# reinterpretcat/qwen3-rs

Hardware: AMD Instinct MI355X
Metric: decode tokens/sec Qwen3-0.6B Q8 g=64 @1 GPU; % of int8 HBM roofline (higher is better)
Workload: dtype i8 (int8 x int8 -> i32 group dots, f32 scales/accumulate); 1 GPU; qwen3-0.6b Q8 group=64 single-stream greedy decode, 8-token prompt, reference generate-mode call pattern (first forward at pos 7, zero KV prefix), ctx 3072, 2751 tokens; mode=reference summation order (bit-identical logits), replicas=1, checkpoint_seed=1234

## Files before the change

qwen3-rs_amd/csrc/q3_attn_short2.h:

```cpp
#if defined(__HIP_DEVICE_COMPILE__) && !defined(__gfx950__)
#error "k_attn_short2 relies on gfx950 s_barrier behaviour for terminated waves; validated on gfx950 only"
#endif
constexpr int kS2Threads = 512;
constexpr int kS2MaxT = 256;
__host__ __device__ inline size_t attn_short2_smem_bytes(int hd, int max_t) { return 4 * (size_t)max_t * (size_t)(hd + 4); }

template <int V> struct IntC { static constexpr int value = V; };

#ifdef Q3_DEV
#define ATT2_STAMP(i, thr) do { if (a.stamps != nullptr && (a.debug & 64) == 0 && blockIdx.x == 3 && (int)threadIdx.x == (thr)) a.stamps[i] = __builtin_amdgcn_s_memtime(); } while (0)
#else
#define ATT2_STAMP(i, thr) do { } while (0)
#endif

template <int HD>
__global__ __launch_bounds__(kS2Threads) void k_attn_short2(const AttnArgs a) {
    static_assert(HD == 128, "head dim instantiated");
    constexpr int NQ4 = HD / 4;
    constexpr int HALF = HD / 2;
    constexpr int LD = HD + 4;
    constexpr int VT = 64;
    extern __shared__ __attribute__((aligned(16))) float ptile[];
    float* const vtile = ptile + VT * LD;
    __shared__ __attribute__((aligned(16))) float q_s[HD];
    __shared__ __attribute__((aligned(16))) float sq_s[2 * HD];
    __shared__ __attribute__((aligned(16))) float att[kS2MaxT];
    __shared__ __attribute__((aligned(16))) float att_e[kS2MaxT];
    __shared__ __attribute__((aligned(16))) float att_p[kS2MaxT];
    __shared__ unsigned long long etab[32];
    __shared__ unsigned vflag;
    __shared__ unsigned bcount;
    ATT2_STAMP(0, 0);
    KSTAMP_BEGIN(a);
    Q3_PIN_S(a.st); Q3_PIN_S(a.pos_override); Q3_PIN_S(a.q); Q3_PIN_S(a.k_raw); Q3_PIN_S(a.key_cache); Q3_PIN_S(a.value_cache);
    Q3_PIN_S(a.q_norm_w); Q3_PIN_S(a.k_norm_w); Q3_PIN_S(a.rope); Q3_PIN_S(a.xb); Q3_PIN_S(a.n_heads); Q3_PIN_S(a.n_kv_heads);
    Q3_PIN_S(a.write_q);

    const int kv_mul = a.kv_mul, xq = (int)((blockIdx.x * a.kvh_magic) >> 20);
    const int kvh = (int)blockIdx.x - xq * a.n_kv_heads;
    const int h = kvh * kv_mul + xq;
    const int tid = threadIdx.x, lane = tid & 63;
    const int wave = __builtin_amdgcn_readfirstlane(tid >> 6);
    const size_t kvd = (size_t)a.n_kv_heads * HD;
    const int pos_v = a.pos_override >= 0 ? a.pos_override : a.st->pos;
    const float* kbase = a.key_cache + (size_t)kvh * HD;
    const float* vbase = a.value_cache + (size_t)kvh * HD;

    if (wave == 4 || wave == 5) {
        const int pos = __builtin_amdgcn_readfirstlane(pos_v);
        const int np = pos + 1;
        const bool vsplit = gridDim.y == 2 && np > 64;
        if (gridDim.y == 2 && blockIdx.y == 1 && np <= 64) return;
        if (vsplit && wave == 5) {
            __syncthreads();
            __syncthreads();
            if (np > 128) __syncthreads();
            __syncthreads();
            return;
        }
        const int e = vsplit ? 64 * (int)blockIdx.y + lane : 64 * (wave - 4) + lane;
        const unsigned eoff = 4u * (unsigned)e;
        float vv[kShortVSets][32];
        auto v_issue = [&](float (&R)[32], int c) {
#pragma unroll
            for (int u = 0; u < 32; ++u) R[u] = *(const float*)((const char*)(vbase + (size_t)min(32 * c + u, pos) * kvd) + eoff);
        };
        auto v_pull = [&](float (&R)[32], int c) {
            const float* vp = vtile + e;
#pragma unroll
            for (int u = 0; u < 32; ++u) R[u] = vp[min(32 * c + u, pos) * HD];
        };
        const bool vlds = np <= VT;
        if (tid == 256) { vflag = 0u; bcount = 0u; }
        if (!vlds) {
#pragma unroll
            for (int c = 0; c < 2; ++c) v_issue(vv[c], c);
        }
        __syncthreads();
        if (!vlds) {
#pragma unroll
            for (int c = 2; c < kShortVSets; ++c)
                if (32 * c < np) v_issue(vv[c], c);
        }
        __syncthreads();
        if (vlds) {
            while (__hip_atomic_load(&vflag, __ATOMIC_ACQUIRE, __HIP_MEMORY_SCOPE_WORKGROUP) < 4u) __builtin_amdgcn_s_sleep(1);
#pragma unroll
            for (int c = 0; c < VT / 32; ++c)
                if (32 * c < np) v_pull(vv[c], c);
        }
        if (np > 128) __syncthreads();
        __syncthreads();
        ATT2_STAMP(5, 256);
        const v4f e4 = ((const v4f*)att_e)[lane];
        float sum;
        if (np <= 128) {
            sum = seq_chain(-0.0f, (const v4f*)att_e, (((np + 3) >> 2) + 7) & ~7);
        } else {
            const float etot = (e4.x + e4.y) + (e4.z + e4.w);
            sum = spec_sum_lanes(etot, (np + 3) >> 2, [&](float s) { return chain4(s, e4); });
        }
        ATT2_STAMP(13, 256);
        const float inv = 1.0f / sum;
        v4f p4;
        p4.x = e4.x * inv; p4.y = e4.y * inv; p4.z = e4.z * inv; p4.w = e4.w * inv;
        ((v4f*)att_p)[lane] = p4;
        wave_lds_sync();
        float o = 0.0f;
        auto fold_chunk = [&](const float (&R)[32], int c) {
            const v4f* pp = (const v4f*)att_p + 8 * c;
            v4f pq[8];
#pragma unroll
            for (int u4 = 0; u4 < 8; ++u4) pq[u4] = pp[u4];
#pragma unroll
            for (int u4 = 0; u4 < 8; ++u4) {
                if (32 * c + 4 * u4 < np) {
                    const v4f pv = pq[u4];
                    const v2f t01 = (v2f){pv.x, pv.y} * (v2f){R[4 * u4 + 0], R[4 * u4 + 1]};
                    const v2f t23 = (v2f){pv.z, pv.w} * (v2f){R[4 * u4 + 2], R[4 * u4 + 3]};
                    o = o + t01.x;
                    o = o + t01.y;
                    o = o + t23.x;
                    o = o + t23.y;
                }
            }
        };
#pragma unroll
        for (int c = 0; c < kShortVSets; ++c)
            if (32 * c < np) fold_chunk(vv[c], c);
        for (int c = kShortVSets; 32 * c < np; c += 2) {
            v_issue(vv[0], c);
            if (32 * (c + 1) < np) v_issue(vv[1], c + 1);
            fold_chunk(vv[0], c);
            if (32 * (c + 1) < np) fold_chunk(vv[1], c + 1);
        }
        ATT2_STAMP(14, 256);
        a.xb[(size_t)h * HD + e] = o;
        if (a.xbq != nullptr) {
            const float m = group_max_f32(fabsf(o), a.xb_group);
            const float scale = m / 127.0f;
            const int qv = (scale != 0.0f) ? quant_round_i8(o / scale) : 0;
            const int idx = h * HD + e;
            a.xbq[idx] = (int8_t)qv;
            if ((idx & (a.xb_group - 1)) == 0) a.xbs[idx / a.xb_group] = scale;
        }
        ATT2_STAMP(6, 256);
        KSTAMP_END(a);
        return;
    }

    int pos, np;
    if (wave < 2) {
        const bool is_q = wave == 0;
        const float* rawp = is_q ? a.q + (size_t)h * HD : a.k_raw + (size_t)kvh * HD;
        const float r_lo = rawp[lane], r_hi = rawp[lane + HALF];
        const float* nw = is_q ? a.q_norm_w : a.k_norm_w;
        const float w_lo = nw[lane], w_hi = nw[lane + HALF];
        __builtin_amdgcn_sched_barrier(0);
        pos = __builtin_amdgcn_readfirstlane(pos_v);
        np = pos + 1;
        if (gridDim.y == 2 && blockIdx.y == 1 && np <= 64) return;
        const v2f cs = *(const v2f*)(a.rope + (size_t)pos * HD + 2 * lane);
        ATT2_STAMP(1, 0);
        float* sq = sq_s + (is_q ? 0 : HD);
        sq[lane] = r_lo * r_lo;
        sq[lane + HALF] = r_hi * r_hi;
        wave_lds_sync();
        const float ss = seq_chain(-0.0f, (const v4f*)sq, NQ4);
        const float f = 1.0f / sqrtf(ss / (float)HD + kEps);
        const float xv = w_lo * (f * r_lo);
        const float yv = w_hi * (f * r_hi);
        const float a0 = xv * cs.x, b0 = yv * cs.y;
        const float a1 = xv * cs.y, b1 = yv * cs.x;
        const float lo = a0 - b0, hi = a1 + b1;
        if (is_q) {
            q_s[lane] = lo;
            q_s[lane + HALF] = hi;
            if (a.write_q) {
                a.q[(size_t)h * HD + lane] = lo;
                a.q[(size_t)h * HD + lane + HALF] = hi;
            }
        } else if ((h % kv_mul) == 0 && blockIdx.y == 0) {
            float* krow = a.key_cache + (size_t)pos * kvd + (size_t)kvh * HD;
            krow[lane] = lo;
            krow[lane + HALF] = hi;
        }
        ATT2_STAMP(2, 0);
        __syncthreads();
        if (!is_q) {
            ptile[pos * LD + lane] = q_s[lane] * lo;
            ptile[pos * LD + lane + HALF] = q_s[lane + HALF] * hi;
        }
    } else {
        unsigned long long etv = 0ull;
        if (wave == 7 && lane < 32) etv = kExp2Tab[lane];
#ifdef Q3_DEV
        const int hint = a.row_steps;
#else
        constexpr int hint = 0;
#endif
        if (hint <= 0) {
            pos = __builtin_amdgcn_readfirstlane(pos_v);
            np = pos + 1;
            if (gridDim.y == 2 && blockIdx.y == 1 && np <= 64) return;
        }
        ATT2_STAMP(8, 128);
        const int sidx = 64 * ((wave & 1) + (wave >= 6 ? 2 : 0)) + lane;
        const int r0 = sidx >> 5, col = sidx & 31;
        const unsigned loff = 4u * ((unsigned)r0 * (unsigned)kvd + 4u * (unsigned)col);
        const int kmax = max(a.seq_len / 8 - 1, 0);
        float* lp = ptile + r0 * LD + 4 * col;
        float* lv = vtile + r0 * HD + 4 * col;
        auto stage = [&](auto tier, auto with_v) {
            constexpr int T = decltype(tier)::value;
            constexpr bool V = decltype(with_v)::value != 0;
            v4f rk[T], rv[V ? T : 1];
#pragma unroll
            for (int k = 0; k < T; ++k) rk[k] = *(const v4f*)((const char*)(kbase + (size_t)min(k, kmax) * 8 * kvd) + loff);
            __builtin_amdgcn_sched_barrier(0);
            if constexpr (V) {
#pragma unroll
                for (int k = 0; k < T; ++k) rv[k] = *(const v4f*)((const char*)(vbase + (size_t)min(k, kmax) * 8 * kvd) + loff);
            }
            ATT2_STAMP(9, 128);
            if (hint > 0) {
                pos = __builtin_amdgcn_readfirstlane(pos_v);
                np = pos + 1;
            }
            __syncthreads();
            const v4f qv = ((const v4f*)q_s)[col];
#pragma unroll
            for (int k = 0; k < T; ++k) {
                const v2f p01 = (v2f){qv.x, qv.y} * (v2f){rk[k].x, rk[k].y};
                const v2f p23 = (v2f){qv.z, qv.w} * (v2f){rk[k].z, rk[k].w};
                v4f pr; pr.x = p01.x; pr.y = p01.y; pr.z = p23.x; pr.w = p23.y;
                if (r0 + 8 * k < pos) *(v4f*)(lp + 8 * k * LD) = pr;
            }
            if (wave == 7 && lane < 32) etab[lane] = etv;
            ATT2_STAMP(11, 128);
            if constexpr (V) {
                __syncthreads();
#pragma unroll
                for (int k = 0; k < T; ++k)
                    if (r0 + 8 * k < np) *(v4f*)(lv + 8 * k * HD) = rv[k];
                __builtin_amdgcn_fence(__ATOMIC_RELEASE, "workgroup");
                if (lane == 0) __hip_atomic_fetch_add(&vflag, 1u, __ATOMIC_RELAXED, __HIP_MEMORY_SCOPE_WORKGROUP);
                ATT2_STAMP(10, 128);
            }
        };
        const int tn = hint > 0 ? hint : (pos + 8) >> 3;
        if (tn <= 1) stage(IntC<1>{}, IntC<1>{});
        else if (tn <= 2) stage(IntC<2>{}, IntC<1>{});
        else if (tn <= 3) stage(IntC<3>{}, IntC<1>{});
        else if (tn <= 4) stage(IntC<4>{}, IntC<1>{});
        else if (tn <= 6) stage(IntC<6>{}, IntC<1>{});
        else if (tn <= 8) stage(IntC<8>{}, IntC<1>{});
        else if (tn <= 12) stage(IntC<12>{}, IntC<0>{});
        else if (tn <= 16) stage(IntC<16>{}, IntC<0>{});
        else if (tn <= 24) stage(IntC<24>{}, IntC<0>{});
        else stage(IntC<32>{}, IntC<0>{});
        if (np <= VT) return;
        __syncthreads();
        if (wave >= 6 || np <= 128) return;
    }
    if (wave < 2) __syncthreads();
    ATT2_STAMP(3, 0);

    const int t = 64 * wave + lane;
    float sc = -__builtin_inff();
    if (64 * wave < np) {
        const float scale = 1.0f / sqrtf((float)HD);
        const v4f* pr = (const v4f*)(ptile + min(t, pos) * LD);
        float dot = -0.0f;
        v4f pa[8], pb[8];
#pragma unroll
        for (int u = 0; u < 8; ++u) pa[u] = pr[u];
#pragma unroll
        for (int b = 0; b < NQ4 / 8; ++b) {
            if (b + 1 < NQ4 / 8) {
#pragma unroll
                for (int u = 0; u < 8; ++u) pb[u] = pr[8 * (b + 1) + u];
                __builtin_amdgcn_s_waitcnt(0xC87F);
            } else {
                __builtin_amdgcn_s_waitcnt(0xC07F);
            }
            __builtin_amdgcn_sched_barrier(0);
#pragma unroll
            for (int u = 0; u < 8; ++u) dot = chain4(dot, pa[u]);
            __builtin_amdgcn_sched_barrier(0);
#pragma unroll
            for (int u = 0; u < 8; ++u) pa[u] = pb[u];
        }
        sc = t < np ? dot * scale : -__builtin_inff();
    }
    const bool one_wave = np <= 64;
    float m;
    if (!one_wave) {
        att[t] = sc;
        if (np <= 128) {
            att[t + 128] = -__builtin_inff();
            __builtin_amdgcn_fence(__ATOMIC_RELEASE, "workgroup");
            if (lane == 0) {
                __hip_atomic_fetch_add(&bcount, 1u, __ATOMIC_RELAXED, __HIP_MEMORY_SCOPE_WORKGROUP);
                while (__hip_atomic_load(&bcount, __ATOMIC_RELAXED, __HIP_MEMORY_SCOPE_WORKGROUP) < 2u) __builtin_amdgcn_s_sleep(1);
            }
            __builtin_amdgcn_fence(__ATOMIC_ACQUIRE, "workgroup");
        } else {
            __syncthreads();
        }
        ATT2_STAMP(4, 0);
        const v4f s4 = ((const v4f*)att)[lane];
        m = fmaxf(fmaxf(s4.x, s4.y), fmaxf(s4.z, s4.w));
    } else {
        ATT2_STAMP(4, 0);
        m = sc;
    }
    m = group_max_f32(m, 64);
    float ev = 0.0f;
    if (64 * wave < np) {
        ev = q3_expf_wave(t < np ? sc - m : 0.0f, etab);
        ev = t < np ? ev : 0.0f;
    }
    att_e[t] = ev;
    if (np <= 128) att_e[t + 128] = 0.0f;
    __syncthreads();
    KSTAMP_END(a);
}
```

Measured before the change: 1130 tokens/s.

## Software-pipeline attention PV fold and exact-length softmax sum in short kernel

Restructures the short-context attention PV accumulation into a compile-time walk. Products for the next V chunk are computed while the previous chunk's sequential add chain runs, and probability loads and late V loads are issued ahead with explicit waitcnt and sched barriers. The softmax denominator now uses an exact-length sequential chain with a handled remainder and double-buffered LDS reads, where before it was padded to a multiple of eight. The q write-back is moved to the kernel tail and limited to blockIdx.y==0. This aims to hide LDS and global load latency and trim wasted adds, at the cost of more registers and more code complexity.

```diff
diff --git a/qwen3-rs_amd/csrc/q3_attn_short2.h b/qwen3-rs_amd/csrc/q3_attn_short2.h
--- a/qwen3-rs_amd/csrc/q3_attn_short2.h
+++ b/qwen3-rs_amd/csrc/q3_attn_short2.h
@@ -6,6 +6,56 @@
 __host__ __device__ inline size_t attn_short2_smem_bytes(int hd, int max_t) { return 4 * (size_t)max_t * (size_t)(hd + 4); }
 
 template <int V> struct IntC { static constexpr int value = V; };
+
+template <int MAXB>
+__device__ __forceinline__ float seq_chain_rem(float s, const v4f* p, int nq) {
+    const int nb = nq >> 3;
+    const v4f* pw = p + (nq & 7);
+    v4f buf[2][8];
+    auto head = [&](auto tc) {
+        constexpr int T = decltype(tc)::value;
+        v4f h[T > 0 ? T : 1];
+#pragma unroll
+        for (int k = 0; k < T; ++k) h[k] = p[k];
+        if (nb > 0) {
+#pragma unroll
+            for (int k = 0; k < 8; ++k) buf[0][k] = pw[k];
+            if constexpr (T > 0) __builtin_amdgcn_s_waitcnt(0xC87F);
+        } else {
+            __builtin_amdgcn_s_waitcnt(0xC07F);
+        }
+        __builtin_amdgcn_sched_barrier(0);
+#pragma unroll
+        for (int k = 0; k < T; ++k) s = chain4(s, h[k]);
+        __builtin_amdgcn_sched_barrier(0);
+    };
+    switch (nq & 7) {
+    case 1: head(IntC<1>{}); break;
+    case 2: head(IntC<2>{}); break;
+    case 3: head(IntC<3>{}); break;
+    case 4: head(IntC<4>{}); break;
+    case 5: head(IntC<5>{}); break;
+    case 6: head(IntC<6>{}); break;
+    case 7: head(IntC<7>{}); break;
+    default: head(IntC<0>{}); break;
+    }
+#pragma unroll
+    for (int i = 0; i < MAXB; ++i) {
+        if (i >= nb) break;
+        if (i + 1 < MAXB && i + 1 < nb) {
+#pragma unroll
+            for (int k = 0; k < 8; ++k) buf[(i + 1) & 1][k] = pw[8 * (i + 1) + k];
+            __builtin_amdgcn_s_waitcnt(0xC87F);
+        } else {
+            __builtin_amdgcn_s_waitcnt(0xC07F);
+        }
+        __builtin_amdgcn_sched_barrier(0);
+#pragma unroll
+        for (int k = 0; k < 8; ++k) s = chain4(s, buf[i & 1][k]);
+        __builtin_amdgcn_sched_barrier(0);
+    }
+    return s;
+}
 
 #ifdef Q3_DEV
 #define ATT2_STAMP(i, thr) do { if (a.stamps != nullptr && (a.debug & 64) == 0 && blockIdx.x == 3 && (int)threadIdx.x == (thr)) a.stamps[i] = __builtin_amdgcn_s_memtime(); } while (0)
@@ -95,7 +145,7 @@
         const v4f e4 = ((const v4f*)att_e)[lane];
         float sum;
         if (np <= 128) {
-            sum = seq_chain(-0.0f, (const v4f*)att_e, (((np + 3) >> 2) + 7) & ~7);
+            sum = seq_chain_rem<4>(-0.0f, (const v4f*)att_e, (np + 3) >> 2);
         } else {
             const float etot = (e4.x + e4.y) + (e4.z + e4.w);
             sum = spec_sum_lanes(etot, (np + 3) >> 2, [&](float s) { return chain4(s, e4); });
@@ -107,33 +157,95 @@
         ((v4f*)att_p)[lane] = p4;
         wave_lds_sync();
         float o = 0.0f;
-        auto fold_chunk = [&](const float (&R)[32], int c) {
-            const v4f* pp = (const v4f*)att_p + 8 * c;
-            v4f pq[8];
-#pragma unroll
-            for (int u4 = 0; u4 < 8; ++u4) pq[u4] = pp[u4];
+        const int nsets = (np + 31) >> 5;
+        const int last4 = (np - 32 * (nsets - 1) + 3) >> 2;
+        v4f pq[8];
+        auto p_request = [&](int c) {
+#pragma unroll
+            for (int u4 = 0; u4 < 8; ++u4) pq[u4] = ((const v4f*)att_p)[8 * c + u4];
+        };
+        auto products = [&](float (&R)[32]) {
+            __builtin_amdgcn_s_waitcnt(0xC07F);
+            __builtin_amdgcn_sched_barrier(0);
+            v2f t[16];
 #pragma unroll
             for (int u4 = 0; u4 < 8; ++u4) {
-                if (32 * c + 4 * u4 < np) {
-                    const v4f pv = pq[u4];
-                    const v2f t01 = (v2f){pv.x, pv.y} * (v2f){R[4 * u4 + 0], R[4 * u4 + 1]};
-                    const v2f t23 = (v2f){pv.z, pv.w} * (v2f){R[4 * u4 + 2], R[4 * u4 + 3]};
-                    o = o + t01.x;
-                    o = o + t01.y;
-                    o = o + t23.x;
-                    o = o + t23.y;
+                t[2 * u4 + 0] = (v2f){pq[u4].x, pq[u4].y} * (v2f){R[4 * u4 + 0], R[4 * u4 + 1]};
+                t[2 * u4 + 1] = (v2f){pq[u4].z, pq[u4].w} * (v2f){R[4 * u4 + 2], R[4 * u4 + 3]};
+            }
+            asm volatile("" : "+v"(o) : "v"(t[0]), "v"(t[1]), "v"(t[2]), "v"(t[3]), "v"(t[4]), "v"(t[5]), "v"(t[6]), "v"(t[7]),
+                         "v"(t[8]), "v"(t[9]), "v"(t[10]), "v"(t[11]), "v"(t[12]), "v"(t[13]), "v"(t[14]), "v"(t[15]));
+#pragma unroll
+            for (int u2 = 0; u2 < 16; ++u2) { R[2 * u2] = t[u2].x; R[2 * u2 + 1] = t[u2].y; }
+        };
+        auto chain = [&](const float (&R)[32], auto n4) {
+            __builtin_amdgcn_sched_barrier(0);
+#pragma unroll
+            for (int u = 0; u < 4 * decltype(n4)::value; ++u) o = o + R[u];
+            __builtin_amdgcn_sched_barrier(0);
+        };
+        auto chain_last = [&](const float (&R)[32]) {
+            switch (last4) {
+            case 1: chain(R, IntC<1>{}); break;
+            case 2: chain(R, IntC<2>{}); break;
+            case 3: chain(R, IntC<3>{}); break;
+            case 4: chain(R, IntC<4>{}); break;
+            case 5: chain(R, IntC<5>{}); break;
+            case 6: chain(R, IntC<6>{}); break;
+            case 7: chain(R, IntC<7>{}); break;
+            default: chain(R, IntC<8>{}); break;
+            }
+        };
+        auto v_issue_late = [&](float (&R)[32], int c) {
+#pragma unroll
+            for (int u = 0; u < 32; ++u) {
+                typedef const __attribute__((address_space(1))) char* gchar_p;
+                gchar_p row = (gchar_p)(vbase + (size_t)min(32 * c + u, pos) * kvd);
+                asm volatile("" : "+s"(row));
+                R[u] = *(const __attribute__((address_space(1))) float*)(row + eoff);
+            }
+        };
+        auto far = [&]() {
+            constexpr int c = kShortVSets - 1;
+            v_issue_late(vv[0], c + 1);
+            if (c + 2 < nsets) v_issue_late(vv[1], c + 2);
+            chain(vv[c], IntC<8>{});
+            if (c + 3 < nsets) v_issue_late(vv[2], c + 3);
+            products(vv[0]);
+            if (c + 2 < nsets) {
+                p_request(c + 2); products(vv[1]);
+                chain(vv[0], IntC<8>{});
+                if (c + 3 < nsets) {
+                    p_request(c + 3); products(vv[2]);
+                    chain(vv[1], IntC<8>{});
+                    chain_last(vv[2]);
+                } else {
+                    chain_last(vv[1]);
                 }
-            }
-        };
-#pragma unroll
-        for (int c = 0; c < kShortVSets; ++c)
-            if (32 * c < np) fold_chunk(vv[c], c);
-        for (int c = kShortVSets; 32 * c < np; c += 2) {
-            v_issue(vv[0], c);
-            if (32 * (c + 1) < np) v_issue(vv[1], c + 1);
-            fold_chunk(vv[0], c);
-            if (32 * (c + 1) < np) fold_chunk(vv[1], c + 1);
-        }
+            } else {
+                chain_last(vv[0]);
+            }
+        };
+        auto walk = [&](auto self, auto cc) -> void {
+            constexpr int c = decltype(cc)::value;
+            static_assert(kS2MaxT / 32 == kShortVSets + 3 && kShortVSets == 5, "three sets behind five register sets");
+            if (c + 1 < nsets) {
+                if constexpr (c + 1 < kShortVSets) {
+                    products(vv[c + 1]);
+                    p_request(c + 2);
+                    chain(vv[c], IntC<8>{});
+                    self(self, IntC<c + 1>{});
+                } else {
+                    far();
+                }
+                return;
+            }
+            chain_last(vv[c]);
+        };
+        p_request(0);
+        products(vv[0]);
+        p_request(1);
+        walk(walk, IntC<0>{});
         ATT2_STAMP(14, 256);
         a.xb[(size_t)h * HD + e] = o;
         if (a.xbq != nullptr) {
@@ -150,6 +262,7 @@
     }
 
     int pos, np;
+    float q_lo = 0.0f, q_hi = 0.0f;
     if (wave < 2) {
         const bool is_q = wave == 0;
         const float* rawp = is_q ? a.q + (size_t)h * HD : a.k_raw + (size_t)kvh * HD;
@@ -176,10 +289,7 @@
         if (is_q) {
             q_s[lane] = lo;
             q_s[lane + HALF] = hi;
-            if (a.write_q) {
-                a.q[(size_t)h * HD + lane] = lo;
-                a.q[(size_t)h * HD + lane + HALF] = hi;
-            }
+            q_lo = lo; q_hi = hi;
         } else if ((h % kv_mul) == 0 && blockIdx.y == 0) {
             float* krow = a.key_cache + (size_t)pos * kvd + (size_t)kvh * HD;
             krow[lane] = lo;
@@ -324,5 +434,9 @@
     att_e[t] = ev;
     if (np <= 128) att_e[t + 128] = 0.0f;
     __syncthreads();
+    if (wave == 0 && a.write_q && blockIdx.y == 0) {
+        a.q[(size_t)h * HD + lane] = q_lo;
+        a.q[(size_t)h * HD + lane + HALF] = q_hi;
+    }
     KSTAMP_END(a);
 }
```

Result: no change. 1132 tokens/s (median of 4 runs) (+0.2%).
